# allenai/gpv-1

Measured on AMD Instinct MI355X. Metric: images/sec/node (train step, 480x640, bs32/GPU), higher is better.
Workload: dtype bf16; 1 GPU; GPV-1 (ResNet-50 + 6+6 DETR layers, 100 queries, RoI head, BERT-base, 3 co-attention, 3 text-decoder layers, V=10000) CocoCaptioning-only train step, dropout 0.1, AdamW; global_batch=32, image=480x640, parallelism=dp1

## Files before the change

### gpv-1_amd/csrc/gemm_glds_tt.hip

```cpp
#include "gemm_common.h"

namespace gpvk {
namespace {


typedef __attribute__((address_space(3))) void lds_void_t;
typedef const __attribute__((address_space(1))) void glb_void_t;

__device__ __forceinline__ bf16x8 tr_frag(const unsigned char* p) {
  typedef short __attribute__((ext_vector_type(4))) s16x4;
  typedef __attribute__((address_space(3))) s16x4 lds_s16x4;
  s16x4 a = __builtin_amdgcn_ds_read_tr16_b64_v4i16((lds_s16x4*)(p));
  s16x4 b = __builtin_amdgcn_ds_read_tr16_b64_v4i16((lds_s16x4*)(p + 4 * ROWBYTES));
  typedef short __attribute__((ext_vector_type(8))) s16x8;
  s16x8 r = {a[0], a[1], a[2], a[3], b[0], b[1], b[2], b[3]};
  return __builtin_bit_cast(bf16x8, r);
}

template <bool CONV, int ABL = 0>
__device__ __forceinline__ void glds_tt_core(const GemmK& p, int tile, int ksplit) {
  extern __shared__ __attribute__((aligned(256))) unsigned char smem[];
  const int tid = threadIdx.x, lane = tid & 63, wave = tid >> 6;
  const int wm = wave >> 1, wn = wave & 1;
  const ConvGeom& g = p.cg;
// ... 541 lines not shown
        for (int j = 0; j < 2; ++j) acc[i0 + i][j0 + j] = mfma16(bfr[j][kk], af[i][kk], acc[i0 + i][j0 + j]);
    __builtin_amdgcn_s_setprio(0);
    __builtin_amdgcn_sched_barrier(0);
    __builtin_amdgcn_s_barrier();
    asm volatile("" ::: "memory");
    __builtin_amdgcn_sched_barrier(0);
  };
#define W8H_READ_A(SLOT)                                                                       \
  _Pragma("unroll") for (int i = 0; i < 4; ++i) {                                              \
    af[i][0] = tr_frag_asm<(SLOT) * W8_HALF>(a_sl[i] + bufo);                                  \
    af[i][1] = tr_frag_asm<(SLOT) * W8_HALF + 32 * ROWBYTES>(a_sl[i] + bufo);                  \
  }
#define W8H_READ_B(SLOT)                                                                       \
  _Pragma("unroll") for (int j = 0; j < 2; ++j) {                                              \
    bfr[j][0] = tr_frag_asm<(SLOT) * W8_HALF>(b_sl[j] + bufo);                                 \
    bfr[j][1] = tr_frag_asm<(SLOT) * W8_HALF + 32 * ROWBYTES>(b_sl[j] + bufo);                 \
  }

  issue01(0, 0); issue2(0, 0); issue01(1, 1); issue2(1, 1);
  asm volatile("s_waitcnt vmcnt(8)" ::: "memory");
  __builtin_amdgcn_s_barrier();
  if (wm == 1) __builtin_amdgcn_s_barrier();
  asm volatile("" ::: "memory");

  int buf = 0, buf2 = 2;
  for (int t = 0; t < nkt; ++t) {
    const uint32_t bufo = buf * W8H_BUF;
    W8H_READ_B(1)
    W8H_READ_A(0)
    __builtin_amdgcn_sched_barrier(0);
    issue01(t + 2, buf2);
    asm volatile("s_waitcnt vmcnt(10)" ::: "memory");
    mma(0, 0);
    if constexpr (BH == 2) { W8H_READ_B(2) } else { W8H_READ_A(2) }
    __builtin_amdgcn_sched_barrier(0);
    issue2(t + 2, buf2);
    asm volatile("s_waitcnt vmcnt(8)" ::: "memory");
    if constexpr (BH == 2) mma(0, 2); else mma(4, 0);
    buf = buf == 2 ? 0 : buf + 1;
    buf2 = buf2 == 2 ? 0 : buf2 + 1;
  }
#undef W8H_READ_A
#undef W8H_READ_B
  if (wm == 0) __builtin_amdgcn_s_barrier();
  asm volatile("s_waitcnt vmcnt(0)" ::: "memory");

  const bool direct = p.ws == nullptr;
  float* Cp = direct ? reinterpret_cast<float*>(p.C) : p.ws + (int64_t)ksplit * p.M * p.N;
  const int64_t cpitch = direct ? p.ldc : p.N;
#pragma unroll
  for (int i = 0; i < NI; ++i) {
    const int m = row0 + (i >> 2) * 128 + wm * 64 + (i & 3) * 16 + li;
    const float rs = p.rowscale ? p.rowscale[m] * p.alpha : p.alpha;
#pragma unroll
    for (int j = 0; j < NJ; ++j) {
      if (!hval[j >> 1]) continue;
      const int n = col0 + (j >> 1) * 128 + wn * 32 + (j & 1) * 16 + fg * 4;
      float4* dst = reinterpret_cast<float4*>(Cp + (int64_t)m * cpitch + n);
      float4 v = make_float4(acc[i][j][0] * rs, acc[i][j][1] * rs, acc[i][j][2] * rs, acc[i][j][3] * rs);
      if (direct) { const float4 c = *dst; v.x += c.x; v.y += c.y; v.z += c.z; v.w += c.w; }
      *dst = v;
    }
  }
}

template <bool CONV>
__device__ __forceinline__ void glds_tt_body(const GemmK& p) {
  const int gx = gridDim.x, nwg = gx * (int)gridDim.y, bid = (int)blockIdx.x + gx * (int)blockIdx.y;
  const int v = xcd_contiguous(bid, nwg);
  const int ksplit = v / gx;
  glds_tt_core<CONV>(p, v - ksplit * gx, ksplit);
}
__global__ __launch_bounds__(256) void glds_wgrad_kernel(GemmK p) { glds_tt_body<true>(p); }
__global__ __launch_bounds__(256) void glds_tt_kernel(GemmK p) { glds_tt_body<false>(p); }

struct GroupK {
  int n;
  int tile_start[GPV_TT_GROUP_MAX + 1];
  gpv_tt_problem prob[GPV_TT_GROUP_MAX];
};
static_assert(sizeof(GroupK) <= 4096, "kernel argument segment");

__global__ __launch_bounds__(256) void glds_tt_group_kernel(GroupK g) {
  const int bid = blockIdx.x;
  int pi = 0;
  while (pi + 1 < g.n && bid >= g.tile_start[pi + 1]) ++pi;
  const gpv_tt_problem& q = g.prob[pi];
  GemmK p{};
  p.A = q.A; p.B = q.B; p.C = q.C; p.a_rowsum = q.a_rowsum;
  p.M = q.M; p.N = q.N; p.K = q.K; p.lda = q.lda; p.ldb = q.ldb; p.ldc = q.ldc;
  p.alpha = 1.0f; p.ws = nullptr;
  p.tilesN = q.N / TBN;
  p.kt_per_split = (q.K + TBK - 1) / TBK;
  glds_tt_core<false>(p, bid - g.tile_start[pi], 0);
}

struct WgProb {
  const void* A; const void* B; float* C; const float* rowscale;
  int M, N, K, lda, ldc;
  int kt_per_split, tilesN, tiles;
  int unit_start;
  int direct;
  int64_t ws_off;
  int IH, IW, Cs, Cin, OH, OW, KH, KW, SH, SW, PH, PW;
};
static_assert(sizeof(WgProb) == 128, "descriptor size");
constexpr int WG_MAX = 28;
struct WgGroupK { int n; int pad; float* ws; WgProb prob[WG_MAX]; };
static_assert(sizeof(WgGroupK) <= 4096, "kernel argument segment");

template <int ABL>
__device__ __forceinline__ void wgrad_group_body(const WgGroupK& g) {
  const int nwg = gridDim.x, bid = blockIdx.x;
  const int v = xcd_contiguous(bid, nwg);
  int pi = 0;
  while (pi + 1 < g.n && v >= g.prob[pi + 1].unit_start) ++pi;
  const WgProb& q = g.prob[pi];
  GemmK p{};
  p.A = q.A; p.B = q.B; p.C = q.C; p.rowscale = q.rowscale;
  p.M = q.M; p.N = q.N; p.K = q.K; p.lda = q.lda; p.ldb = 0; p.ldc = q.ldc;
  p.alpha = 1.0f;
  p.ws = q.direct ? nullptr : g.ws + q.ws_off;
  p.tilesN = q.tilesN; p.kt_per_split = q.kt_per_split;
  p.cg.IH = q.IH; p.cg.IW = q.IW; p.cg.Cs = q.Cs; p.cg.Cin = q.Cin; p.cg.OH = q.OH; p.cg.OW = q.OW;
  p.cg.KH = q.KH; p.cg.KW = q.KW; p.cg.SH = q.SH; p.cg.SW = q.SW; p.cg.PH = q.PH; p.cg.PW = q.PW;
  const int u = v - q.unit_start;
  const int ksplit = u / q.tiles;
  glds_tt_core<true, ABL>(p, u - ksplit * q.tiles, ksplit);
}
__global__ __launch_bounds__(256) void glds_wgrad_group_kernel(WgGroupK g) { wgrad_group_body<0>(g); }
__global__ __launch_bounds__(512) void wg8_group_kernel(WgGroupK g) {
  const int nwg = gridDim.x, bid = blockIdx.x;
  const int v = xcd_contiguous(bid, nwg);
  int pi = 0;
  while (pi + 1 < g.n && v >= g.prob[pi + 1].unit_start) ++pi;
  const WgProb& q = g.prob[pi];
  GemmK p{};
  p.A = q.A; p.B = q.B; p.C = q.C; p.rowscale = q.rowscale;
  p.M = q.M; p.N = q.N; p.K = q.K; p.lda = q.lda; p.ldb = 0; p.ldc = q.ldc;
  p.alpha = 1.0f;
  p.ws = q.direct ? nullptr : g.ws + q.ws_off;
  p.tilesN = q.tilesN; p.kt_per_split = q.kt_per_split;
  p.cg.IH = q.IH; p.cg.IW = q.IW; p.cg.Cs = q.Cs; p.cg.Cin = q.Cin; p.cg.OH = q.OH; p.cg.OW = q.OW;
  p.cg.KH = q.KH; p.cg.KW = q.KW; p.cg.SH = q.SH; p.cg.SW = q.SW; p.cg.PH = q.PH; p.cg.PW = q.PW;
  const int u = v - q.unit_start;
  const int ksplit = u / q.tiles;
  wg8_core<true>(p, u - ksplit * q.tiles, ksplit);
}
__global__ __launch_bounds__(512) void wg8h_group_kernel(WgGroupK g) {
  const int nwg = gridDim.x, bid = blockIdx.x;
  const int v = xcd_contiguous(bid, nwg);
  int pi = 0;
  while (pi + 1 < g.n && v >= g.prob[pi + 1].unit_start) ++pi;
  const WgProb& q = g.prob[pi];
  GemmK p{};
  p.A = q.A; p.B = q.B; p.C = q.C; p.rowscale = q.rowscale;
  p.M = q.M; p.N = q.N; p.K = q.K; p.lda = q.lda; p.ldb = 0; p.ldc = q.ldc;
  p.alpha = 1.0f;
  p.ws = (q.direct & 1) ? nullptr : g.ws + q.ws_off;
  p.tilesN = q.tilesN; p.kt_per_split = q.kt_per_split;
  p.cg.IH = q.IH; p.cg.IW = q.IW; p.cg.Cs = q.Cs; p.cg.Cin = q.Cin; p.cg.OH = q.OH; p.cg.OW = q.OW;
  p.cg.KH = q.KH; p.cg.KW = q.KW; p.cg.SH = q.SH; p.cg.SW = q.SW; p.cg.PH = q.PH; p.cg.PW = q.PW;
  const int u = v - q.unit_start;
  const int ksplit = u / q.tiles;
  if (q.direct & 2) wg8h_core<2, 1>(p, u - ksplit * q.tiles, ksplit);
  else wg8h_core<1, 2>(p, u - ksplit * q.tiles, ksplit);
}
#ifdef GPV_TUNING
__global__ __launch_bounds__(256) void glds_wgrad_group_abl1_kernel(WgGroupK g) { wgrad_group_body<1>(g); }
__global__ __launch_bounds__(256) void glds_wgrad_group_abl2_kernel(WgGroupK g) { wgrad_group_body<2>(g); }
__global__ __launch_bounds__(256) void glds_wgrad_group_abl3_kernel(WgGroupK g) { wgrad_group_body<3>(g); }
__global__ __launch_bounds__(256) void glds_wgrad_group_abl4_kernel(WgGroupK g) { wgrad_group_body<4>(g); }
__global__ __launch_bounds__(256) void glds_wgrad_group_abl5_kernel(WgGroupK g) { wgrad_group_body<5>(g); }
__global__ __launch_bounds__(256) void glds_wgrad_group_abl6_kernel(WgGroupK g) { wgrad_group_body<6>(g); }
#endif

constexpr int W8L_PMAX = GPV_TT_GROUP_MAX, W8L_GMAX = 200;
// ... 10 lines not shown
__global__ __launch_bounds__(512) void wg8_tt_group_kernel(W8LGroupK g) {
  const int bid = blockIdx.x, xcd = bid & 7, loc = bid >> 3;
  if (loc >= g.cnt[xcd]) return;
  const int v = xcd * g.Q + loc;
  int lo = 0, hi = g.n_grp - 1;
  while (lo < hi) {
    const int mid = (lo + hi + 1) >> 1;
    if ((int)g.grp[mid].v_start <= v) lo = mid; else hi = mid - 1;
  }
  const W8LGrp gr = g.grp[lo];
  const W8LProb& q = g.prob[gr.prob];
  GemmK p{};
  p.A = q.A; p.B = q.B; p.C = q.C; p.a_rowsum = q.a_rowsum;
  p.M = q.MN / q.N; p.N = q.N; p.K = q.K; p.lda = q.lda; p.ldb = q.ldb; p.ldc = q.ldc;
  p.alpha = 1.0f;
  p.ws = q.ws_off < 0 ? nullptr : g.ws + q.ws_off;
  p.tilesN = q.N / 256; p.kt_per_split = q.kt_per_split;
  wg8_core<false>(p, v - gr.v_start, gr.slice);
}

struct WgRed { const float* ws; float* C; int64_t MN; int split, N, ldc, blk_start; };
struct WgRedK { int n; int pad; WgRed r[WG_MAX]; };

__global__ __launch_bounds__(256) void wgrad_group_reduce_kernel(WgRedK g) {
  const int bid = blockIdx.x;
  int pi = 0;
  while (pi + 1 < g.n && bid >= g.r[pi + 1].blk_start) ++pi;
  const WgRed& q = g.r[pi];
  const int64_t idx = (int64_t)(bid - q.blk_start) * 256 + threadIdx.x;
  if (idx * 4 >= q.MN) return;
  const int nq = q.N >> 2;
  const int m = (int)(idx / nq), c4 = (int)(idx - (int64_t)m * nq);
  const float* src = q.ws + (int64_t)m * q.N + c4 * 4;
  float4 a = {0.f, 0.f, 0.f, 0.f};
#pragma unroll 4
  for (int sidx = 0; sidx < q.split; ++sidx) {
    const float4 v = *reinterpret_cast<const float4*>(src + (int64_t)sidx * q.MN);
    a.x += v.x; a.y += v.y; a.z += v.z; a.w += v.w;
  }
  float4* dst = reinterpret_cast<float4*>(q.C + (int64_t)m * q.ldc + c4 * 4);
  float4 c = *dst;
  c.x += a.x; c.y += a.y; c.z += a.z; c.w += a.w;
  *dst = c;
}

template <typename F>
int launch_tt(F fn, const GemmK& k, const Route& r, bool& attr_done, hipStream_t st) {
  GemmK p = k;
  p.kt_per_split = r.kt_per_split;
  p.ws = reinterpret_cast<float*>(k.ws_base);
  p.tilesN = r.tilesN;
  if (!attr_done) {
    hipError_t e = hipFuncSetAttribute(reinterpret_cast<const void*>(fn), hipFuncAttributeMaxDynamicSharedMemorySize, (int)r.lds);
    if (e != hipSuccess) { (void)hipGetLastError(); return (int)e; }
    attr_done = true;
  }
  hipLaunchKernelGGL(fn, dim3(r.gx, r.gy, r.gz), dim3(r.block), (size_t)r.lds, st, p);
  GPV_CHECK_LAUNCH();
  return launch_splitk_reduce(p.ws, r.split, p.M, p.N, reinterpret_cast<float*>(p.C), p.ldc, st);
}

}

int glds_tt_launch(const GemmK& k, const Route& r, hipStream_t st) {
  static bool attr_done[2] = {false, false};
  if (r.family == FAM_GLDS_WGRAD) return launch_tt(glds_wgrad_kernel, k, r, attr_done[0], st);
  return launch_tt(glds_tt_kernel, k, r, attr_done[1], st);
}

}

extern "C" int gpv_gemm_tt_group(const gpv_tt_problem* problems, int n, void* stream) {
  using namespace gpvk;
  if (!problems || n <= 0) return (int)hipErrorInvalidValue;
  static bool attr_done = false;
  constexpr int lds = 2 * TSTAGE;
  if (!attr_done) {
    hipError_t e = hipFuncSetAttribute(reinterpret_cast<const void*>(glds_tt_group_kernel), hipFuncAttributeMaxDynamicSharedMemorySize, lds);
    if (e != hipSuccess) { (void)hipGetLastError(); return (int)e; }
    attr_done = true;
  }
  for (int i0 = 0; i0 < n; i0 += GPV_TT_GROUP_MAX) {
    GroupK g{};
    g.n = n - i0 < GPV_TT_GROUP_MAX ? n - i0 : GPV_TT_GROUP_MAX;
    int tiles = 0;
    for (int i = 0; i < g.n; ++i) {
      const gpv_tt_problem& q = problems[i0 + i];
      if (!q.A || !q.B || !q.C || q.M <= 0 || q.N <= 0 || q.K <= 0 || q.M % TBM != 0 || q.N % TBN != 0 || q.lda % 8 != 0 ||
          q.ldb % 8 != 0 || q.ldc % 4 != 0 || !al16(q.A) || !al16(q.B) || !al16(q.C) ||
          (int64_t)q.K * q.lda >= (1ll << 30) || (int64_t)q.K * q.ldb >= (1ll << 30))
        return (int)hipErrorInvalidValue;
      g.prob[i] = q;
      g.tile_start[i] = tiles;
      tiles += (q.M / TBM) * (q.N / TBN);
    }
    g.tile_start[g.n] = tiles;
    hipLaunchKernelGGL(glds_tt_group_kernel, dim3(tiles), dim3(256), lds, reinterpret_cast<hipStream_t>(stream), g);
    GPV_CHECK_LAUNCH();
  }
  return 0;
}

extern "C" int gpv_conv_wgrad_group(const gpv_conv_wgrad_problem* probs, int n, void* workspace, int64_t workspace_bytes, void* stream) {
  using namespace gpvk;
  if (!probs || n <= 0) return (int)hipErrorInvalidValue;
  hipStream_t st = reinterpret_cast<hipStream_t>(stream);
  static const int target_kt = [] { const int v = tune_env("GPV_WGRAD_GROUP_KT", 150); return v < 8 ? 8 : v; }();
  static bool attr_done = false;
  constexpr int lds = 2 * TSTAGE;
  typedef void (*wg_fn)(WgGroupK);
#ifdef GPV_TUNING
  static const int abl = tune_env("GPV_WG_ABL", 0);
  const wg_fn fn = abl == 1 ? glds_wgrad_group_abl1_kernel : abl == 2 ? glds_wgrad_group_abl2_kernel : abl == 3 ? glds_wgrad_group_abl3_kernel : abl == 4 ? glds_wgrad_group_abl4_kernel : abl == 5 ? glds_wgrad_group_abl5_kernel : abl == 6 ? glds_wgrad_group_abl6_kernel
                                                                                                        : glds_wgrad_group_kernel;
#else
  const wg_fn fn = glds_wgrad_group_kernel;
#endif
  if (!attr_done) {
    hipError_t e = hipFuncSetAttribute(reinterpret_cast<const void*>(fn), hipFuncAttributeMaxDynamicSharedMemorySize, lds);
    if (e != hipSuccess) { (void)hipGetLastError(); return (int)e; }
    attr_done = true;
  }
  static bool attr8_done = false;
  if (!attr8_done) {
    hipError_t e = hipFuncSetAttribute(reinterpret_cast<const void*>(wg8_group_kernel), hipFuncAttributeMaxDynamicSharedMemorySize, W8_LDS);
    if (e != hipSuccess) { (void)hipGetLastError(); return (int)e; }
    attr8_done = true;
  }
  static const int target_kt8 = [] { const int v = tune_env("GPV_WG8_KT", 150); return v < 8 ? 8 : v; }();
  auto eligible8 = [&](const gpv_conv_wgrad_problem& q) {
    const int64_t K64 = (int64_t)q.B * q.OH * q.OW;
    return q.Cout % 256 == 0 && q.Cin % 256 == 0 && q.Cs % 8 == 0 && al16(q.dy) && al16(q.x) && al16(q.dw) &&
           TBK / q.OW + 2 <= q.OH && (int64_t)q.IH * q.IW * q.Cs * q.B < (1ll << 30) && K64 * q.Cout < (1ll << 30) && K64 >= 8 * TBK;
  };
  static bool attr8h_done = false;
  if (!attr8h_done) {
    hipError_t e = hipFuncSetAttribute(reinterpret_cast<const void*>(wg8h_group_kernel), hipFuncAttributeMaxDynamicSharedMemorySize, W8H_LDS);
    if (e != hipSuccess) { (void)hipGetLastError(); return (int)e; }
    attr8h_done = true;
  }
  static const int forced_kt8h = tune_env("GPV_WG8H_KT", 0);
  static const int ramp_kt8h = tune_env("GPV_WG8H_C", 15);
  auto eligible8h = [&](const gpv_conv_wgrad_problem& q) {
    const int64_t K64 = (int64_t)q.B * q.OH * q.OW;
    return g_knobs.wg8h != 0 && q.Cout % 128 == 0 && q.Cin % 128 == 0 && q.Cs % 8 == 0 && al16(q.dy) && al16(q.x) && al16(q.dw) &&
           TBK / q.OW + 2 <= q.OH && (int64_t)q.IH * q.IW * q.Cs * q.B < (1ll << 30) && K64 * q.Cout < (1ll << 30) && K64 >= 8 * TBK;
  };
  bool use8 = g_knobs.wg8 != 0;
  if (use8 && g_knobs.wg8 == 1) {
    int64_t u8 = 0;
    for (int i = 0; i < n; ++i) {
      const gpv_conv_wgrad_problem& q = probs[i];
      if (!eligible8(q)) continue;
      const int64_t kt = ((int64_t)q.B * q.OH * q.OW + TBK - 1) / TBK;
      u8 += (int64_t)(q.Cout / 256) * (q.KH * q.KW * q.Cin / 256) * ((kt + target_kt8 / 2) / target_kt8 > 0 ? (kt + target_kt8 / 2) / target_kt8 : 1);
    }
    use8 = u8 >= 128;
  }
  int target_kt8h = forced_kt8h >= 8 ? forced_kt8h : 150;
  if (forced_kt8h < 8 && g_knobs.wg8h != 0) {
    int64_t best = -1;
    for (int kt = 64; kt <= 640; kt += 4) {
      int64_t u = 0;
      int longest = 0;
      for (int i = 0; i < n; ++i) {
        const gpv_conv_wgrad_problem& q = probs[i];
        if ((use8 && eligible8(q)) || !eligible8h(q)) continue;
        const int M = q.Cout, N = q.KH * q.KW * q.Cin;
        const int kt_total = (int)(((int64_t)q.B * q.OH * q.OW + TBK - 1) / TBK);
        int split = (kt_total + kt / 2) / kt;
        if (split < 1) split = 1;
        const int kps = (kt_total + split - 1) / split;
        split = (kt_total + kps - 1) / kps;
        u += (int64_t)(M % 256 == 0 ? (M / 256) * (N / 128) : (M / 128) * ((N + 255) / 256)) * split;
        if (kps > longest) longest = kps;
      }
      if (u == 0) break;
      const int64_t cost = ((u + 255) / 256) * (longest + ramp_kt8h);
      if (best < 0 || cost < best) { best = cost; target_kt8h = kt; }
    }
// ... 206 lines not shown
```

### gpv-1_amd/csrc/gemm_route.h

```cpp
#pragma once
#include <stdint.h>
#include "../../include/gpv_hip.h"
#include "host_defs.h"

namespace gpvk {

enum { OP_PLAIN = 0, OP_TRANS = 1, OP_CONV = 2 };

struct ConvGeom {
  int IH, IW, Cs, Cin, OH, OW, KH, KW, SH, SW, PH, PW, dgrad;
  int cm;
  int cls_rows;
};

struct GemmK {
  const void* A; const void* B; void* C;
  int M, N, K;
  int64_t lda, ldb, ldc, sA, sB, sC;
  float alpha;
  const float* rowscale; const float* bias;
  const void* res; int64_t ldr, sR;
  const void* mask; int64_t ldm;
  int act; uint32_t dthresh; float dscale; uint64_t seed; const uint64_t* seed_dev;
  int accumulate, split_k, kt_per_split, tilesN;
  int vecA, vecB;
  int conv1x1;
  int depi;
  int no_small;
  int nt_io;
  void* ws_base; int64_t ws_bytes;
  float* ws;
  const uint32_t* mask_bits;
  uint32_t* out_bits;
  float* a_rowsum;
  ConvGeom cg;
};

constexpr int BK = 32;
constexpr int LDK = 40;
constexpr int GBK = 64;
constexpr int ROWB = 128;
constexpr int GBM = 256;
constexpr int PIPE_THREADS = 512;
constexpr int SBM = 64, SBN = 64, SBK = 128, SPITCH = SBK + 8;
constexpr int TPITCH = SBN + 16;
constexpr int TBM = 128, TBN = 128, TBK = 64;
constexpr int ROWBYTES = 256;
constexpr int OP_BYTES = TBK * ROWBYTES;
constexpr int TSTAGE = 2 * OP_BYTES;
constexpr int C3_OOB = 0x7ffffff0;
constexpr int C3_NSL = 64;
struct PipeCfg { int bm, bn, wm, ns; };
constexpr PipeCfg kCfgs[] = {{256, 128, 4, 3}, {192, 128, 4, 3}, {128, 128, 2, 3}, {160, 256, 2, 3}, {128, 256, 2, 3}, {96, 256, 2, 3},
                             {64, 64, 2, 6}, {32, 64, 2, 8}};
constexpr int kNumBig = 6;
constexpr int kNumCfgs = sizeof(kCfgs) / sizeof(kCfgs[0]);
inline int c1s_cols(int K, int N) {
  const int cap = K <= 128 ? 512 : (K == 256 ? 256 : 128);
  return N < cap ? N : cap;
}

struct Knobs {
  int glds = tune_env("GPV_GLDS", 1);
  int pipe = tune_env("GPV_PIPE", 1);
  int pipe_small = tune_env("GPV_PIPE_SMALL", 1);
  int skinny = 1;
  int gemv = 1;
  int c1s = 1;
  int c3s = 1;
  int halo = tune_env("GPV_C3_HALO", 1);
  int wgrad = tune_env("GPV_GLDS_WGRAD", 1);
  int wg8 = tune_env("GPV_WG8", 1);
  int wg8h = tune_env("GPV_WG8H", 1);
  int w8l = tune_env("GPV_W8L", 0);
  int two_per_cu = tune_env("GPV_TWO_PER_CU", 1);
  int bm96_fill = tune_env("GPV_BM96", 1);
  int skinny_tile = tune_env("GPV_SKINNY_TILE", 0);
  long n_glds = 0, n_pipe = 0, n_halo = 0, n_c1s = 0, n_c3s = 0, n_gemv = 0, n_wg8 = 0;
  bool forced() const { return glds >= 2 || pipe >= 100; }
};
extern Knobs g_knobs;

enum Family {
  FAM_GEMV, FAM_C1S, FAM_C3S, FAM_CONV_SPLIT, FAM_PIPE, FAM_SKINNY, FAM_GLDS, FAM_HALO, FAM_GLDS_WGRAD, FAM_GLDS_TT, FAM_SKINNY_TT,
  FAM_TILE, FAM_S2_FILL
};
inline const char* family_name(int f) {
  static const char* const names[] = {"gemv", "c1s", "c3s", "conv_split", "pipe", "skinny", "glds", "halo", "glds_wgrad", "glds_tt", "skinny_tt",
                                      "tile", "s2_fill"};
  return names[f];
}

struct Route {
  int family;
  int amode, bmode;
  int dt_in, dt_out;
  int bm, bn;
  int cfg;
  int vec;
  int c11, nt;
  int ck, nh, np;
  int res, mask, lin, bits;
  int dgrad, d2, waves;
  unsigned gx, gy, gz, block;
  int64_t lds;
  int tilesN, split, kt_per_split;
  int two_pass;
  int depi;
  int ncols;
  int rows, nstrip, nseg, nitems;
};

constexpr int kRouteInvalid = 1;

struct Routed {
  int err;
  int nparts, batch;
  GemmK k[2];
  Route r[2];
};

inline int two_per_cu_bm(const GemmK& k, int batch, const Knobs& kn) {
  if (k.N % 128 != 0 || batch != 1) return 0;
  if (kn.bm96_fill && k.M <= 1024) {
    const int64_t t128 = (int64_t)((k.M + 127) / 128) * (k.N / 128), t96 = (int64_t)((k.M + 95) / 96) * (k.N / 128);
    if (t96 <= 256 && t96 * 10 >= t128 * 12) return 96;
  }
  int best = 0;
  double best_u = 0.0;
  const int heights[] = {160, 96};
  for (int bm : heights) {
    const int64_t t = (int64_t)((k.M + bm - 1) / bm) * (k.N / 128);
    if (t <= 384) continue;
    const double u = (double)t / (512.0 * ((t + 511) / 512));
    if ((t <= 512 || u >= 0.9) && u > best_u) { best = bm; best_u = u; }
  }
  return best;
}
inline bool glds_two_per_cu(const GemmK& k, int batch, const Knobs& kn) {
  return kn.two_per_cu && k.K >= 512 && (!k.cg.cm || k.cg.KH == 1) && two_per_cu_bm(k, batch, kn) != 0;
}

inline bool gemv_select(const GemmK& k, int dtype_in, int dtype_out, int batch, const Knobs& kn, Route* r) {
  if (kn.gemv == 0 || kn.forced() || k.M > 8 || batch != 1 || k.accumulate || k.split_k > 1) return false;
  if (k.rowscale || k.mask || k.dthresh || k.a_rowsum) return false;
  if (k.M > 2 && k.N >= 4096) return false;
  if (k.K % 8 != 0 || k.lda % 8 != 0 || k.ldb % 8 != 0 || !al16(k.A) || !al16(k.B)) return false;
  if (!((dtype_in == GPV_BF16 && (dtype_out == GPV_BF16 || dtype_out == GPV_F32)) || (dtype_in == GPV_F32 && dtype_out == GPV_F32))) return false;
  r->family = FAM_GEMV; r->dt_in = dtype_in; r->dt_out = dtype_out;
  r->bm = k.M == 1 ? 1 : (k.M == 2 ? 2 : (k.M <= 4 ? 4 : 8));
  r->bn = k.N >= 4096 ? 4 : (k.N >= 2048 ? 2 : 1);
  r->gx = (unsigned)((k.N + 4 * r->bn - 1) / (4 * r->bn)); r->gy = r->gz = 1; r->block = 256; r->lds = 0;
  return true;
}

inline bool c1s_select(const GemmK& k, int dtype_in, int dtype_out, bool linear, const Knobs& kn, Route* r) {
  static const int env = tune_env("GPV_C1S", -1);
// ... 533 lines not shown
      k.cg = ConvGeom{};
      k.cg.SH = k.cg.SW = 1;
      k.conv1x1 = 1;
      {
        static const int64_t nt_min = (int64_t)tune_env("GPV_NT_MIN_MB", 200) << 20;
        k.nt_io = (int64_t)k.M * k.N * esz >= nt_min ? 1 : 0;
      }
      k.vecA = al16(a->x) && (a->Cs % vecel == 0) && (int64_t)k.M * a->Cs * esz < 0x7ffffff0ll ? 1 : 0;
      c.amode = OP_PLAIN;
      if (want_bits) {
        if (!k.vecA) return route_fail(out, kRouteInvalid);
        k.out_bits = reinterpret_cast<uint32_t*>(a->y_mask_bits);
        k.mask_bits = reinterpret_cast<const uint32_t*>(a->relu_mask_bits);
        if (k.mask_bits) { k.mask = a->relu_mask_bits; k.ldm = a->Cout; }
        if (!route_try(&k, c, fam(FAM_C1S), kn, r)) route_fail(out, kRouteInvalid);
        return;
      }
      if (!route_try(&k, c, (k.vecA ? fam(FAM_C1S) : 0u) | (k.M <= 8192 && !kn.forced() ? fam(FAM_SKINNY) : 0u) | kDldsTiles, kn, r)) route_fail(out, kRouteInvalid);
      return;
    }
    static const bool s2_split = tune_env("GPV_S2_DGRAD_SPLIT", 1) != 0;
    if (s2_split && a->mode == 1 && k.cg.cm && a->KH == 1 && a->KW == 1 && a->PH == 0 && a->PW == 0 && a->dtype_in == GPV_BF16 &&
        a->dtype_out == GPV_BF16 && a->Cout % 8 == 0 && al16(a->y) && (!a->res || al16(a->res)) &&
        (!a->relu_mask || al16(a->relu_mask)) && k.vecA && k.vecB) {
      out->k[1] = k;
      k.M = k.cg.cls_rows;
      if (!route_try(&k, c, kDldsTiles, kn, r)) return route_fail(out, kRouteInvalid);
      Route& f = out->r[1];
      f = Route{};
      f.family = FAM_S2_FILL; f.dt_in = f.dt_out = GPV_BF16;
      f.ncols = a->Cout / 8;
      f.gx = (unsigned)(((int64_t)a->B * a->OH * a->OW * f.ncols + 255) / 256); f.gy = f.gz = 1; f.block = 256;
      out->nparts = 2;
      return;
    }
    if (want_bits) {
      if (!(a->KH == 3 && a->KW == 3 && k.vecA && k.vecB)) return route_fail(out, kRouteInvalid);
      k.mask_bits = reinterpret_cast<const uint32_t*>(a->relu_mask_bits);
      k.mask = a->relu_mask_bits; k.ldm = a->Cout;
      if (!route_try(&k, c, fam(FAM_C3S), kn, r)) route_fail(out, kRouteInvalid);
      return;
    }
    const bool vec = k.vecA && k.vecB;
    c.ws = a->workspace; c.ws_bytes = a->workspace_bytes;
    if (!route_try(&k, c, (a->KH == 3 && a->KW == 3 && vec ? fam(FAM_C3S) : 0u) | (vec && a->mode == 0 && a->workspace ? fam(FAM_CONV_SPLIT) : 0u) |
                              (vec ? fam(FAM_PIPE) | fam(FAM_GLDS) : 0u) | fam(FAM_TILE), kn, r)) route_fail(out, kRouteInvalid);
    return;
  }
  if (a->mode == 2) {
    if (a->dtype_out != GPV_F32) return route_fail(out, kRouteInvalid);
    if (a->Cin % 64 != 0) return route_fail(out, kRouteInvalid);
    k.A = a->w ; k.B = a->x; k.C = a->y ;
    k.M = a->Cout; k.N = T * a->Cin; k.K = a->B * a->OH * a->OW;
    k.lda = a->Cout; k.ldb = 0; k.ldc = k.N;
    k.accumulate = 1;
    int split = a->split_k;
    if (split < 1) {
      const int kt = (k.K + BK - 1) / BK;
      int64_t want;
      if (a->workspace && a->Cin % 128 == 0 && k.M >= 128) {
        const int64_t t128 = (int64_t)((k.M + 127) / 128) * (k.N / 128);
        want = (544 + t128 / 2) / t128;
        if (want > 288) want = 288;
        while (want > 1 && want * (int64_t)k.M * k.N * 4 > a->workspace_bytes) --want;
      } else {
        const int64_t tiles = (int64_t)((k.M + 63) / 64) * ((k.N + 63) / 64);
        want = 1536 / (tiles > 0 ? tiles : 1);
      }
      if (want > kt / 8) want = kt / 8;
      split = want < 1 ? 1 : (int)want;
    }
    k.split_k = split;
    if (split <= 1) { k.accumulate = 0; k.res = a->y; k.ldr = k.ldc; }
    k.ws_base = a->workspace; k.ws_bytes = a->workspace ? a->workspace_bytes : 0;
    k.vecA = al16(a->w) && (a->Cout % vecel == 0) ? 1 : 0;
    k.vecB = al16(a->x) && (a->Cs % vecel == 0) ? 1 : 0;
    c.amode = OP_TRANS; c.bmode = OP_CONV;
    if (!route_try(&k, c, fam(FAM_GLDS_WGRAD) | fam(FAM_TILE), kn, r)) route_fail(out, kRouteInvalid);
    return;
  }
  route_fail(out, kRouteInvalid);
}

}
```

### gpv-1_amd/transformer.py

```python
import os

import torch
import torch.nn as nn

from . import ops
from .ops import W

HOIST_KV = os.environ.get('GPV_HOIST_KV', '1') != '0'


class LinearP(nn.Module):

    def __init__(self, in_features, out_features, bias=True):
        super().__init__()
        ref = nn.Linear(in_features, out_features, bias=bias)
        self.weight = nn.Parameter(ref.weight.detach().clone())
        self.bias = nn.Parameter(ref.bias.detach().clone()) if bias else None
        self.in_features, self.out_features = in_features, out_features

    def forward(self, x, act=ops.ACT_NONE, drop_p=0.0, out_f32=False, chain=None):
        return ops.linear(x, W(self.weight, self.bias), act, drop_p, out_f32, chain)


def ffn_block(x, l1, l2, norm, drop_p, pos=None, pos_param=None):
    return ops.ffn_block(x, W(l1.weight, l1.bias), W(l2.weight, l2.bias), norm.weight, norm.bias, norm.eps, drop_p, pos, pos_param)


class LayerNormP(nn.Module):
    def __init__(self, dim, eps=1e-5):
        super().__init__()
        self.weight = nn.Parameter(torch.ones(dim))
        self.bias = nn.Parameter(torch.zeros(dim))
        self.eps = eps

    def forward(self, x, s=None, drop_p=0.0, chain=None, pos=None, pos_param=None):
        return ops.add_layernorm(x, s, self.weight, self.bias, self.eps, drop_p, chain, pos, pos_param)

    def proj(self, x, a, lin, drop_p=0.0, chain=None, pos=None, pos_param=None):
        w = W(lin.weight, lin.bias)
        if ops.proj_layernorm_ok(w, x) and (pos is None or ops.LN_POS):
            return ops.proj_add_layernorm(x, a, w, self.weight, self.bias, self.eps, drop_p, chain, pos, pos_param)
        return self.forward(x, lin(a), drop_p, chain, pos, pos_param)


class MultiheadAttention(nn.Module):

    def __init__(self, embed_dim, num_heads, dropout=0.0):
        super().__init__()
        self.embed_dim, self.num_heads, self.dropout = embed_dim, num_heads, dropout
        self.head_dim = embed_dim // num_heads
        self.in_proj_weight = nn.Parameter(torch.empty(3 * embed_dim, embed_dim))
        self.in_proj_bias = nn.Parameter(torch.zeros(3 * embed_dim))
        self.out_proj = LinearP(embed_dim, embed_dim)
        nn.init.xavier_uniform_(self.in_proj_weight)
        nn.init.constant_(self.out_proj.bias, 0.)

    def forward(self, q_in, k_in, v_in, B, Sq, Sk, key_padding_mask=None, causal=False, chains=(None, None, None), kv=None, out_drop=0.0,
                no_proj=False):
        E = self.embed_dim
        w, b = self.in_proj_weight, self.in_proj_bias
        cq, ck, cv = chains
        if kv is not None:
            k_all, kcol, v_all, vcol, sk, sv = kv
            q = ops.linear(q_in, W(w, b, 0, E), chain=cq)
            if k_all is v_all:
                bufs, roles, sinks = [q, k_all], ((0, 0), (1, kcol), (1, vcol)), (None, sk)
            else:
                bufs, roles, sinks = [q, k_all, v_all], ((0, 0), (1, kcol), (2, vcol)), (None, sk, sv)
            o = ops.attention(bufs, roles, B, self.num_heads, Sq, Sk, self.head_dim, kpm=key_padding_mask,
                              causal=causal, drop_p=self.dropout if self.training else 0.0,
                              sinks=sinks if (sk is not None or sv is not None) else None)
            return o if no_proj else self.out_proj(o, drop_p=out_drop)
        if q_in is k_in and k_in is v_in:
            bufs = [ops.linear(q_in, W(w, b, 0, 3 * E), chain=cq)]
            roles = ((0, 0), (0, E), (0, 2 * E))
        elif q_in is k_in:
            if Sq == Sk and ops.attention_qkv_ok(E, self.num_heads, Sq, causal, B):
                o = ops.attention_qkv(q_in, v_in, W(w, b, 0, 3 * E), B, self.num_heads, Sq, kpm=key_padding_mask,
                                      drop_p=self.dropout if self.training else 0.0, chains=(cq, cv))
                return o if no_proj else self.out_proj(o, drop_p=out_drop)
            bufs = [ops.linear(q_in, W(w, b, 0, 2 * E), chain=cq), ops.linear(v_in, W(w, b, 2 * E, 3 * E), chain=cv)]
            roles = ((0, 0), (0, E), (1, 0))
        elif k_in is v_in:
            bufs = [ops.linear(q_in, W(w, b, 0, E), chain=cq), ops.linear(k_in, W(w, b, E, 3 * E), chain=ck)]
            roles = ((0, 0), (1, 0), (1, E))
        else:
            bufs = [ops.linear(q_in, W(w, b, 0, E), chain=cq), ops.linear(k_in, W(w, b, E, 2 * E), chain=ck),
                    ops.linear(v_in, W(w, b, 2 * E, 3 * E), chain=cv)]
            roles = ((0, 0), (1, 0), (2, 0))
        o = ops.attention(bufs, roles, B, self.num_heads, Sq, Sk, self.head_dim, kpm=key_padding_mask, causal=causal,
                          drop_p=self.dropout if self.training else 0.0)
# ... 24 lines not shown
            qk = ops.add(s2, pos)
        else:
            s2, qk = self.norm1(src, pos=pos)
        src = ops.add(src, self.self_attn(qk, qk, s2, B, S, S, kpm, out_drop=p))
        s2 = self.norm2(src)
        return ops.add(src, self.linear2(self.linear1(s2, ops.ACT_RELU, p), drop_p=p))


class TransformerDecoderLayer(nn.Module):
    def __init__(self, d_model, nhead, dim_feedforward=2048, dropout=0.1):
        super().__init__()
        self.self_attn = MultiheadAttention(d_model, nhead, dropout=dropout)
        self.multihead_attn = MultiheadAttention(d_model, nhead, dropout=dropout)
        self.linear1 = LinearP(d_model, dim_feedforward)
        self.linear2 = LinearP(dim_feedforward, d_model)
        self.norm1 = LayerNormP(d_model)
        self.norm2 = LayerNormP(d_model)
        self.norm3 = LayerNormP(d_model)
        self.p = dropout

    def forward(self, tgt, tgt_qp, memory, mem_pos, qpos, qpos_param, B, Q, S, kpm, mem_chain=None, emit=True, kv=None):
        p = self.p if self.training else 0.0
        ch = ops.grad_chain(tgt)
        o = self.self_attn(tgt_qp, tgt_qp, tgt, B, Q, Q, chains=(None, None, ch), no_proj=True)
        tgt, tq = self.norm1.proj(tgt, o, self.self_attn.out_proj, p, chain=ch, pos=qpos, pos_param=qpos_param)
        a = self.multihead_attn(tq, mem_pos, memory, B, Q, S, kpm, chains=(None, mem_chain, mem_chain), kv=kv, no_proj=True)
        tgt = self.norm2.proj(tgt, a, self.multihead_attn.out_proj, p)
        if not emit:
            return ffn_block(tgt, self.linear1, self.linear2, self.norm3, p), None
        return ffn_block(tgt, self.linear1, self.linear2, self.norm3, p, pos=qpos, pos_param=qpos_param)

    def forward_pre(self, tgt, memory, mem_pos, qpos, qpos_param, B, Q, S, kpm):
        p = self.p if self.training else 0.0
        t2, tq = self.norm1(tgt, pos=qpos, pos_param=qpos_param)
        tgt = ops.add(tgt, self.self_attn(tq, tq, t2, B, Q, Q, out_drop=p))
        t2, tq = self.norm2(tgt, pos=qpos, pos_param=qpos_param)
        tgt = ops.add(tgt, self.multihead_attn(tq, mem_pos, memory, B, Q, S, kpm, out_drop=p))
        t2 = self.norm3(tgt)
        return ops.add(tgt, self.linear2(self.linear1(t2, ops.ACT_RELU, p), drop_p=p))


class TransformerEncoder(nn.Module):
    def __init__(self, make_layer, num_layers, norm=None):
        super().__init__()
        self.layers = nn.ModuleList([make_layer() for _ in range(num_layers)])
        self.norm = norm


class TransformerDecoder(nn.Module):
    def __init__(self, make_layer, num_layers, d_model):
        super().__init__()
        self.layers = nn.ModuleList([make_layer() for _ in range(num_layers)])
        self.norm = LayerNormP(d_model)


class Transformer(nn.Module):
    def __init__(self, d_model=512, nhead=8, num_encoder_layers=6, num_decoder_layers=6, dim_feedforward=2048,
                 dropout=0.1, normalize_before=False, return_intermediate_dec=False):
        super().__init__()
        self.normalize_before = bool(normalize_before)
        self.encoder = TransformerEncoder(lambda: TransformerEncoderLayer(d_model, nhead, dim_feedforward, dropout),
                                          num_encoder_layers, LayerNormP(d_model) if normalize_before else None)
        self.decoder = TransformerDecoder(lambda: TransformerDecoderLayer(d_model, nhead, dim_feedforward, dropout),
                                          num_decoder_layers, d_model)
        self.d_model, self.nhead = d_model, nhead
        for p in self.parameters():
            if p.dim() > 1:
                nn.init.xavier_uniform_(p)

    def forward(self, src, mask, query_embed, pos, need_all_layers):
        B, S, C = src.shape
        Q = query_embed.shape[0]
        kpm = mask.to(torch.uint8).contiguous() if mask is not None else None
        x = src.reshape(B * S, C)
        pe = pos.reshape(B * S, C)
        if self.normalize_before:
            return self._forward_pre(x, pe, kpm, query_embed, B, S, C, Q, need_all_layers)
        if torch.is_grad_enabled() and pe.requires_grad:
            return self._forward_plain(x, pe, kpm, query_embed, B, S, C, Q, need_all_layers)
        if len(self.encoder.layers) == 0:
            xq = ops.add(x, pe)
        else:
            xq = ops.add(x, pe)
            for layer in self.encoder.layers:
                x, xq = layer(x, xq, pe, B, S, kpm)
        memory = ops.boundary(x, 'mem')
        mem_pos = xq
        n = len(self.decoder.layers)
        k_all = v_all = sk = sv = mem_chain = None
        if HOIST_KV and n > 1:
            ca = [l.multihead_attn for l in self.decoder.layers]
            k_all = ops.multi_linear(mem_pos, [W(a.in_proj_weight, a.in_proj_bias, C, 2 * C) for a in ca])
            v_all = ops.multi_linear(memory, [W(a.in_proj_weight, a.in_proj_bias, 2 * C, 3 * C) for a in ca])
            if torch.is_grad_enabled() and k_all.requires_grad:
                sk, sv = ops.GradSink(n), ops.GradSink(n)
        else:
            mem_chain = ops.grad_chain(memory)
        qp = query_embed.detach().to(ops.RT.dtype).contiguous()
        tgt = torch.zeros(B * Q, C, device=src.device, dtype=ops.RT.dtype)
        tq = query_embed.to(ops.RT.dtype).unsqueeze(0).expand(B, Q, C).reshape(B * Q, C)
        outs = []
        for i, layer in enumerate(self.decoder.layers):
            tgt, tq = layer(tgt, tq, memory, mem_pos, qp, query_embed, B, Q, S, kpm, mem_chain, emit=i + 1 < n,
                            kv=None if k_all is None else (k_all, i * C, v_all, i * C, sk, sv))
            if need_all_layers or i == n - 1:
                outs.append(self.decoder.norm(tgt).reshape(B, Q, C))
        return outs, memory.reshape(B, S, C)


def _transformer_forward_pre(self, x, pe, kpm, query_embed, B, S, C, Q, need_all_layers):
    pos_grad = torch.is_grad_enabled() and pe.requires_grad
    pe = ops._as_compute(pe) if pos_grad else ops._pos_rows(pe, C)
    for layer in self.encoder.layers:
        x = layer.forward_pre(x, pe, B, S, kpm, pos_grad)
    if pos_grad:
        memory = self.encoder.norm(x)
        mem_pos = ops.add(memory, pe)
    else:
        memory, mem_pos = self.encoder.norm(x, pos=pe)
    qp = query_embed.detach().to(ops.RT.dtype).contiguous()
    tgt = torch.zeros(B * Q, C, device=x.device, dtype=ops.RT.dtype)
    outs = []
    n = len(self.decoder.layers)
    for i, layer in enumerate(self.decoder.layers):
        tgt = layer.forward_pre(tgt, memory, mem_pos, qp, query_embed, B, Q, S, kpm)
        if need_all_layers or i == n - 1:
            outs.append(self.decoder.norm(tgt).reshape(B, Q, C))
    return outs, memory.reshape(B, S, C)


Transformer._forward_pre = _transformer_forward_pre


def _transformer_forward_plain(self, x, pe, kpm, query_embed, B, S, C, Q, need_all_layers):
    pe = ops._as_compute(pe)
    for layer in self.encoder.layers:
        p = layer.p if layer.training else 0.0
        qk = ops.add(x, pe)
        x = layer.norm1(x, layer.self_attn(qk, qk, x, B, S, S, kpm), p)
        x = ffn_block(x, layer.linear1, layer.linear2, layer.norm2, p)
    memory = x
    mem_pos = ops.add(memory, pe)
    qe = query_embed.to(ops.RT.dtype)
    tgt = torch.zeros(B * Q, C, device=x.device, dtype=ops.RT.dtype)
    outs = []
    n = len(self.decoder.layers)
    for i, layer in enumerate(self.decoder.layers):
        p = layer.p if layer.training else 0.0
        tq = ops.add(tgt, qe)
        tgt = layer.norm1(tgt, layer.self_attn(tq, tq, tgt, B, Q, Q), p)
        tgt = layer.norm2(tgt, layer.multihead_attn(ops.add(tgt, qe), mem_pos, memory, B, Q, S, kpm), p)
        tgt = ffn_block(tgt, layer.linear1, layer.linear2, layer.norm3, p)
        if need_all_layers or i == n - 1:
            outs.append(self.decoder.norm(tgt).reshape(B, Q, C))
    return outs, memory.reshape(B, S, C)


Transformer._forward_plain = _transformer_forward_plain


def build_transformer(args):
    return Transformer(d_model=args.hidden_dim, dropout=args.dropout, nhead=args.nheads,
                       dim_feedforward=args.dim_feedforward, num_encoder_layers=args.num_encoder_layers,
                       num_decoder_layers=args.num_decoder_layers, normalize_before=args.pre_norm,
                       return_intermediate_dec=True)
```

Measured before the change: 2163 images/sec.

## Sort grouped TT GEMM problems by K and add persistent-grid cap

The grouped transposed GEMM launch now orders its problems by descending K-tile count, so the longest tiles are scheduled first. The kernel becomes a grid-stride loop over tiles, with an optional grid cap (off by default) for a persistent-style launch. Separately, the encoder loop can insert boundary markers between layers, controlled by the GPV_WGRAD_FLUSH env var, which by default does not contain 'enc'. The aim is better load balance across problems of different K, at the cost of a small scheduling-logic overhead.

```diff
diff --git a/gpv-1_amd/csrc/gemm_glds_tt.hip b/gpv-1_amd/csrc/gemm_glds_tt.hip
--- a/gpv-1_amd/csrc/gemm_glds_tt.hip
+++ b/gpv-1_amd/csrc/gemm_glds_tt.hip
@@ -647,17 +647,20 @@
 static_assert(sizeof(GroupK) <= 4096, "kernel argument segment");
 
 __global__ __launch_bounds__(256) void glds_tt_group_kernel(GroupK g) {
-  const int bid = blockIdx.x;
+  const int first = blockIdx.x, G = gridDim.x, total = g.tile_start[g.n];
   int pi = 0;
-  while (pi + 1 < g.n && bid >= g.tile_start[pi + 1]) ++pi;
-  const gpv_tt_problem& q = g.prob[pi];
-  GemmK p{};
-  p.A = q.A; p.B = q.B; p.C = q.C; p.a_rowsum = q.a_rowsum;
-  p.M = q.M; p.N = q.N; p.K = q.K; p.lda = q.lda; p.ldb = q.ldb; p.ldc = q.ldc;
-  p.alpha = 1.0f; p.ws = nullptr;
-  p.tilesN = q.N / TBN;
-  p.kt_per_split = (q.K + TBK - 1) / TBK;
-  glds_tt_core<false>(p, bid - g.tile_start[pi], 0);
+  for (int t = first; t < total; t += G) {
+    pi = tt_group_find(g.tile_start, g.n, t, pi);
+    const gpv_tt_problem& q = g.prob[pi];
+    GemmK p{};
+    p.A = q.A; p.B = q.B; p.C = q.C; p.a_rowsum = q.a_rowsum;
+    p.M = q.M; p.N = q.N; p.K = q.K; p.lda = q.lda; p.ldb = q.ldb; p.ldc = q.ldc;
+    p.alpha = 1.0f; p.ws = nullptr;
+    p.tilesN = q.N / TBN;
+    p.kt_per_split = (q.K + TBK - 1) / TBK;
+    if (t != first) __syncthreads();
+    glds_tt_core<false>(p, t - g.tile_start[pi], 0);
+  }
 }
 
 struct WgProb {
@@ -834,20 +837,15 @@
   }
   for (int i0 = 0; i0 < n; i0 += GPV_TT_GROUP_MAX) {
     GroupK g{};
-    g.n = n - i0 < GPV_TT_GROUP_MAX ? n - i0 : GPV_TT_GROUP_MAX;
-    int tiles = 0;
-    for (int i = 0; i < g.n; ++i) {
-      const gpv_tt_problem& q = problems[i0 + i];
-      if (!q.A || !q.B || !q.C || q.M <= 0 || q.N <= 0 || q.K <= 0 || q.M % TBM != 0 || q.N % TBN != 0 || q.lda % 8 != 0 ||
-          q.ldb % 8 != 0 || q.ldc % 4 != 0 || !al16(q.A) || !al16(q.B) || !al16(q.C) ||
-          (int64_t)q.K * q.lda >= (1ll << 30) || (int64_t)q.K * q.ldb >= (1ll << 30))
-        return (int)hipErrorInvalidValue;
-      g.prob[i] = q;
-      g.tile_start[i] = tiles;
-      tiles += (q.M / TBM) * (q.N / TBN);
-    }
-    g.tile_start[g.n] = tiles;
-    hipLaunchKernelGGL(glds_tt_group_kernel, dim3(tiles), dim3(256), lds, reinterpret_cast<hipStream_t>(stream), g);
+    TtGroupPlan pl;
+    if (tt_group_plan(problems + i0, n - i0 < GPV_TT_GROUP_MAX ? n - i0 : GPV_TT_GROUP_MAX, g_knobs.tt_cap, &pl) != 0) return (int)hipErrorInvalidValue;
+    g.n = pl.n;
+    for (int i = 0; i < pl.n; ++i) {
+      g.prob[i] = problems[i0 + pl.order[i]];
+      g.tile_start[i] = pl.tile_start[i];
+    }
+    g.tile_start[pl.n] = pl.tiles;
+    hipLaunchKernelGGL(glds_tt_group_kernel, dim3(pl.grid), dim3(256), lds, reinterpret_cast<hipStream_t>(stream), g);
     GPV_CHECK_LAUNCH();
   }
   return 0;
diff --git a/gpv-1_amd/csrc/gemm_route.h b/gpv-1_amd/csrc/gemm_route.h
--- a/gpv-1_amd/csrc/gemm_route.h
+++ b/gpv-1_amd/csrc/gemm_route.h
@@ -73,6 +73,7 @@
   int wg8 = tune_env("GPV_WG8", 1);
   int wg8h = tune_env("GPV_WG8H", 1);
   int w8l = tune_env("GPV_W8L", 0);
+  int tt_cap = tune_env("GPV_TT_CAP", 0);
   int two_per_cu = tune_env("GPV_TWO_PER_CU", 1);
   int bm96_fill = tune_env("GPV_BM96", 1);
   int skinny_tile = tune_env("GPV_SKINNY_TILE", 0);
@@ -772,4 +773,42 @@
   route_fail(out, kRouteInvalid);
 }
 
-}
+struct TtGroupPlan {
+  int n, tiles, grid;
+  int order[GPV_TT_GROUP_MAX];
+  int tile_start[GPV_TT_GROUP_MAX + 1];
+};
+inline bool tt_problem_ok(const gpv_tt_problem& q) {
+  return q.A && q.B && q.C && q.M > 0 && q.N > 0 && q.K > 0 && q.M % TBM == 0 && q.N % TBN == 0 && q.lda % 8 == 0 && q.ldb % 8 == 0 &&
+         q.ldc % 4 == 0 && al16(q.A) && al16(q.B) && al16(q.C) && (int64_t)q.K * q.lda < (1ll << 30) && (int64_t)q.K * q.ldb < (1ll << 30);
+}
+inline int tt_group_plan(const gpv_tt_problem* problems, int n, int cap, TtGroupPlan* pl) {
+  if (!problems || n <= 0 || n > GPV_TT_GROUP_MAX) return kRouteInvalid;
+  int kt[GPV_TT_GROUP_MAX];
+  int64_t tiles = 0;
+  for (int i = 0; i < n; ++i) {
+    if (!tt_problem_ok(problems[i])) return kRouteInvalid;
+    tiles += (int64_t)(problems[i].M / TBM) * (problems[i].N / TBN);
+    const int k = (problems[i].K + TBK - 1) / TBK;
+    int j = i - 1;
+    while (j >= 0 && kt[j] < k) { kt[j + 1] = kt[j]; pl->order[j + 1] = pl->order[j]; --j; }
+    kt[j + 1] = k; pl->order[j + 1] = i;
+  }
+  if (tiles >= (1ll << 31)) return kRouteInvalid;
+  pl->n = n;
+  int t = 0;
+  for (int i = 0; i < n; ++i) {
+    const gpv_tt_problem& q = problems[pl->order[i]];
+    pl->tile_start[i] = t;
+    t += (q.M / TBM) * (q.N / TBN);
+  }
+  pl->tile_start[n] = pl->tiles = t;
+  pl->grid = cap > 0 && cap < t ? cap : t;
+  return 0;
+}
+GPV_HD int tt_group_find(const int* tile_start, int n, int t, int pi) {
+  while (pi + 1 < n && t >= tile_start[pi + 1]) ++pi;
+  return pi;
+}
+
+}
diff --git a/gpv-1_amd/transformer.py b/gpv-1_amd/transformer.py
--- a/gpv-1_amd/transformer.py
+++ b/gpv-1_amd/transformer.py
@@ -7,6 +7,7 @@
 from .ops import W
 
 HOIST_KV = os.environ.get('GPV_HOIST_KV', '1') != '0'
+ENC_FLUSH = 'enc' in os.environ.get('GPV_WGRAD_FLUSH', 'detr').split(',')
 
 
 class LinearP(nn.Module):
@@ -197,7 +198,9 @@
             xq = ops.add(x, pe)
         else:
             xq = ops.add(x, pe)
-            for layer in self.encoder.layers:
+            for i, layer in enumerate(self.encoder.layers):
+                if ENC_FLUSH and i > 0:
+                    x = ops.boundary(x, 'enc')
                 x, xq = layer(x, xq, pe, B, S, kpm)
         memory = ops.boundary(x, 'mem')
         mem_pos = xq
```

Result: no change. 2157 images/sec (-0.3%).
